# hsalehipour/XLB

Hardware: AMD Instinct MI355X
Metric: MLUPS (million lattice updates/s) D3Q19 BGK, 512^3 per GPU (higher is better)
Workload: dtype f32; 1 GPU; D3Q19 BGK FP32FP32 cavity_halfway 512x512x512 (512^3 per GPU), omega=1.0; decomposition=single GPU

## Files before the change

xlb_amd/csrc/api.hip:

```cpp
#include <cstring>

#include "api_internal.hpp"
#include "comm.hpp"

namespace xlb {

static thread_local std::string g_err;

void set_error(const char* fmt, ...) {
  char buf[1024];
  va_list ap;
  va_start(ap, fmt);
  vsnprintf(buf, sizeof(buf), fmt, ap);
  va_end(ap);
  g_err = buf;
}

int64_t opt(const xlbhip_ctx* c, const char* key, int64_t dflt) {
  auto it = c->opts.find(key);
  return it == c->opts.end() ? dflt : it->second;
}

int lattice_q(int lattice) { return lattice == XLBHIP_D2Q9 ? 9 : (lattice == XLBHIP_D3Q19 ? 19 : (lattice == XLBHIP_D3Q27 ? 27 : 0)); }
int lattice_d(int lattice) { return lattice == XLBHIP_D2Q9 ? 2 : 3; }
// ... 78 lines not shown
  int n = 0;
  XLB_HIP(hipGetDeviceCount(&n));
  XLB_REQUIRE(n > 0, "no HIP device visible");
  XLB_REQUIRE(device >= 0 && device < n, "device %d out of range (have %d)", device, n);
  XLB_HIP(hipSetDevice(device));
  xlbhip_ctx* c = new xlbhip_ctx();
  c->device = device;
  XLB_HIP(hipStreamCreateWithFlags(&c->stream, hipStreamNonBlocking));
  int prio_low = 0, prio_high = 0;
  XLB_HIP(hipDeviceGetStreamPriorityRange(&prio_low, &prio_high));
  XLB_HIP(hipStreamCreateWithPriority(&c->comm_stream, hipStreamNonBlocking, prio_high));
  XLB_HIP(hipEventCreate(&c->ev_a));
  XLB_HIP(hipEventCreate(&c->ev_b));
  XLB_HIP(hipEventCreateWithFlags(&c->ev_edge, hipEventDisableTiming));
  XLB_HIP(hipEventCreateWithFlags(&c->ev_halo, hipEventDisableTiming));
  hipDeviceProp_t p;
  XLB_HIP(hipGetDeviceProperties(&p, device));
  c->compute_units = p.multiProcessorCount;
  c->opts["vec"] = 0;
  c->opts["nt_store"] = 1;
  c->opts["nt_load"] = 1;
  c->opts["plane_pad_bytes"] = 4352;
  c->opts["block_threads"] = 256;
  c->opts["xcd_swizzle"] = 0;
  c->opts["block_tz"] = 0;
  c->opts["overlap"] = 1;
  c->opts["smagorinsky_coef_e6"] = 170000;
  c->opts["fuse2"] = 1;
  c->opts["fuse2_xseg"] = 0;
  c->opts["fuse2_clean"] = 1;
  c->opts["fuse2_cus"] = 0;
  c->opts["fuse2_strips"] = 1;
  c->opts["fuse2_rowmap"] = 0;
  c->opts["fast_bgk"] = 0;
  c->opts["exact_math"] = 0;
  c->opts["external_halo"] = 0;
  c->opts["halo_telemetry"] = 1;
  c->opts["ipc_copy"] = 1;
  c->opts["ipc_timeout_ms"] = 180000;
  c->opts["halo_skip"] = 0;
  c->opts["comm_self_test"] = 0;
  *out = c;
  return 0;
}

int xlbhip_destroy(xlbhip_ctx* c) {
  if (!c) return 0;
  (void)hipSetDevice(c->device);
  (void)hipDeviceSynchronize();
  xlbhip_comm_destroy(c);
  (void)hipEventDestroy(c->ev_a);
  (void)hipEventDestroy(c->ev_b);
  (void)hipEventDestroy(c->ev_edge);
  (void)hipEventDestroy(c->ev_halo);
  for (int i = 0; i < xlbhip_ctx::WAIT_RING; ++i) {
    if (c->ev_w0[i]) (void)hipEventDestroy(c->ev_w0[i]);
    if (c->ev_w1[i]) (void)hipEventDestroy(c->ev_w1[i]);
  }
  (void)hipStreamDestroy(c->stream);
  (void)hipStreamDestroy(c->comm_stream);
  delete c;
  return 0;
}

int xlbhip_sync(xlbhip_ctx* c) {
  XLB_REQUIRE(c, "ctx is null");
// ... 516 lines not shown
```

xlb_amd/csrc/step2_d3q19.hip:

```cpp
#include "step2_launch.hpp"

namespace xlb {

int launch_step2_d3q19_bgk(const Step2Launch& p) {
  XLB_REQUIRE(p.tile_ty == 8 && p.tile_tz == 64, "two-step kernel: only the (8 x 64) tile is built");
  if (p.halo) return p.has_bc ? launch2<D3Q19, 1, 8, 64, true>(p) : launch2<D3Q19, 0, 8, 64, true>(p);
  return p.has_bc ? launch2<D3Q19, 1, 8, 64, false>(p) : launch2<D3Q19, 0, 8, 64, false>(p);
}

int step2_build_clean(const Step2Launch& p, uint8_t* out) {
  XLB_REQUIRE(p.meta && out && p.tile_ty == 8 && (p.tile_tz == 64 || (p.tile_tz == 48 && p.halo == 0)), "clean flags: (8 x 64) / (8 x 48) tiles with meta words only");
  const size_t ghost = (size_t)p.halo * p.ny * p.nz;
  const unsigned tiles = (unsigned)(p.ny / 8) * (unsigned)(p.nz / p.tile_tz);
  const int segs = step2_eff_segments(p), swz = step2_eff_swizzle(p, tiles);
  if (p.tile_tz == 48)
    hipLaunchKernelGGL((k_step2_clean<8, 48, false>), dim3(tiles * (unsigned)segs), dim3(256), 0, p.stream, p.meta, p.tile_order, swz, segs, step2_eff_cap(p), p.x_begin,
                       p.x_count, p.nx, p.ny, p.nz, p.tile_oy, p.tile_oz, out);
  else if (p.halo)
    hipLaunchKernelGGL((k_step2_clean<8, 64, true>), dim3(tiles * (unsigned)segs), dim3(256), 0, p.stream, p.meta + ghost, p.tile_order, swz, segs, step2_eff_cap(p), p.x_begin,
                       p.x_count, p.nx, p.ny, p.nz, p.tile_oy, p.tile_oz, out);
  else
    hipLaunchKernelGGL((k_step2_clean<8, 64, false>), dim3(tiles * (unsigned)segs), dim3(256), 0, p.stream, p.meta, p.tile_order, swz, segs, step2_eff_cap(p), p.x_begin,
                       p.x_count, p.nx, p.ny, p.nz, p.tile_oy, p.tile_oz, out);
  XLB_HIP(hipGetLastError());
  return 0;
}
int step2_items(const Step2Launch& p) { return (p.ny / p.tile_ty) * (p.nz / p.tile_tz) * step2_eff_segments(p); }

}

#ifdef XLB_STEP2_TRACE
extern "C" int xlbhip_debug_step2_trace(unsigned long long* out, int n) {
  constexpr int N = xlb::TRACE_PLANES * xlb::TRACE_WAVES * xlb::TRACE_EVENTS;
  if (n < N) return N;
  if (hipDeviceSynchronize() != hipSuccess) return -1;
  return hipMemcpyFromSymbol(out, HIP_SYMBOL(xlb::g_step2_trace), sizeof(unsigned long long) * N) == hipSuccess ? 0 : -1;
}
#endif
```

xlb_amd/csrc/step2_kernel.hpp:

```cpp
#pragma once
#include "step_kernel.hpp"

namespace xlb {

#ifdef XLB_STEP2_TRACE
constexpr int TRACE_PLANES = 6, TRACE_EVENTS = 8, TRACE_WAVES = 11, TRACE_FIRST = 40, TRACE_BLOCK = 300;
static __device__ unsigned long long g_step2_trace[TRACE_PLANES * TRACE_WAVES * TRACE_EVENTS];
__device__ __forceinline__ void trace_stamp(int d, int e) {
  __builtin_amdgcn_sched_barrier(0);
  unsigned long long tm;
  asm volatile("s_memtime %0\n\ts_waitcnt lgkmcnt(0)" : "=s"(tm)::"memory");
  if (blockIdx.x == TRACE_BLOCK && d >= TRACE_FIRST && d < TRACE_FIRST + TRACE_PLANES && (threadIdx.x & 63) == 0)
    g_step2_trace[((d - TRACE_FIRST) * TRACE_WAVES + (threadIdx.x >> 6)) * TRACE_EVENTS + e] = tm;
  __builtin_amdgcn_sched_barrier(0);
}
#define XLB_TRACE(d, e) trace_stamp(d, e)
#else
#define XLB_TRACE(d, e)
#endif

template <class L>
constexpr int n_cz0() {
  int n = 0;
  for (int l = 0; l < L::Q; ++l) n += L::c(2, l) == 0 ? 1 : 0;
  return n;
}
template <class L>
constexpr int nth_cz(int cz, int k) {
  for (int l = 0; l < L::Q; ++l)
    if (L::c(2, l) == cz && k-- == 0) return l;
  return 0;
}

template <class L, int HASBC, bool SLACK = false>
struct S2Ring {
  static_assert(!SLACK || HASBC == 0, "the slack ring is the BC-free body's");
  static constexpr int group(int l) { return L::c(0, l) + 1; }
  static constexpr int gcount(int g) {
    int n = 0;
    for (int m = 0; m < L::Q; ++m) n += group(m) == g ? 1 : 0;
    return n;
  }
  static constexpr int gidx(int l) {
    int n = 0;
    for (int m = 0; m < l; ++m) n += group(m) == group(l) ? 1 : 0;
    return n;
  }
  static constexpr int glife(int g) { return (g == 0 ? (HASBC != 0 ? 2 : 1) : (g == 1 ? 2 : 3)) + (SLACK ? 1 : 0); }
  template <int life>
  static __device__ __forceinline__ int buf(int q) {
    static_assert(life >= 1 && life <= 4, "ring life");
// ... 26 lines not shown

__device__ __forceinline__ void lds_barrier() { asm volatile("s_waitcnt lgkmcnt(0)\n\ts_barrier" ::: "memory"); }

template <class L>
struct S2Meta {
  static constexpr bool WIDE = L::Q > 24;
  static constexpr unsigned KBITS = WIDE ? 3 : 4, MSHIFT = 2 * KBITS;
  static constexpr unsigned K_HWM = WIDE ? 5u : 15u;
  static __device__ __forceinline__ unsigned kind(unsigned w) { return w & ((1u << KBITS) - 1u); }
  static __device__ __forceinline__ unsigned slot(unsigned w) { return (w >> KBITS) & ((1u << KBITS) - 1u); }
  static __device__ __forceinline__ unsigned missing(unsigned w) { return WIDE ? (w >> MSHIFT) << 1 : w >> MSHIFT; }
};

__device__ __forceinline__ unsigned wave_or(unsigned v) {
  v |= (unsigned)__builtin_amdgcn_update_dpp(0, (int)v, 0x111, 0xf, 0xf, true);
  v |= (unsigned)__builtin_amdgcn_update_dpp(0, (int)v, 0x112, 0xf, 0xf, true);
  v |= (unsigned)__builtin_amdgcn_update_dpp(0, (int)v, 0x114, 0xf, 0xf, true);
  v |= (unsigned)__builtin_amdgcn_update_dpp(0, (int)v, 0x118, 0xf, 0xf, true);
  return (unsigned)__builtin_amdgcn_readlane((int)v, 15) | (unsigned)__builtin_amdgcn_readlane((int)v, 31) |
         (unsigned)__builtin_amdgcn_readlane((int)v, 47) | (unsigned)__builtin_amdgcn_readlane((int)v, 63);
}

template <class T, class S>
__device__ __forceinline__ unsigned slot_of(const StepArgs<T, S>& a, unsigned id) {
  unsigned slot = 0;
#pragma unroll
  for (int s = 0; s < MAX_FAST_BCS; ++s) {
    const unsigned sid = (unsigned)(a.ids_packed >> (8 * s)) & 0xffu;
    slot = (id == sid) ? (unsigned)s : slot;
  }
  return slot;
}

__device__ __forceinline__ void step2_seg_range(int x_begin, int x_count, int n_seg, int x_cap, int seg, int& x_lo, int& x_hi) {
  if (x_cap > 0 && n_seg >= 3) {
    const int inner = x_count - 2 * x_cap, m = n_seg - 2;
    x_lo = seg == 0 ? x_begin : x_begin + x_cap + (int)(((long)inner * (seg - 1)) / m);
    x_hi = seg == 0 ? x_begin + x_cap : (seg == n_seg - 1 ? x_begin + x_count : x_begin + x_cap + (int)(((long)inner * seg) / m));
    if (seg == n_seg - 1) x_lo = x_begin + x_count - x_cap;
  } else {
    x_lo = x_begin + (int)(((long)x_count * seg) / n_seg);
    x_hi = x_begin + (int)(((long)x_count * (seg + 1)) / n_seg);
  }
}

template <class L, class T, class S, int COLL, int HASBC, int TY, int TZ, bool SLAB, int GMAX, bool PIN, bool FAST, bool SLACK = false, int STRIPS = 0>
__device__ __forceinline__ void step2_body(const StepArgs<T, S>& a, S* lds, unsigned* ldsmeta, T* bcval, S* strip_stage = nullptr) {
  using G = S2Geom<L, HASBC, TY, TZ>;
  using R = S2Ring<L, HASBC, SLACK>;
  using M = S2Meta<L>;
  constexpr int Q = L::Q, NE = G::NE, EZ = G::EZ;
  constexpr unsigned ES = sizeof(S);
  constexpr bool SR = (STRIPS & 1) != 0, SW = (STRIPS & 2) != 0;
  static_assert(STRIPS == 0 || STRIPS == 2 || STRIPS == 3 || STRIPS == 4, "STRIPS: 0, 2 (write), 3 (read + write) or 4 (row-aligned lanes only)");
  static_assert(STRIPS == 0 || (TZ == 64 && sizeof(S) == 4), "strip buffers: (TY x 64) tiles, 4-byte store type");
  static_assert(sizeof(S) == 4, "k_step2 keeps f(t+1) as 4-byte store values in LDS");
  auto ring = [&](auto lc, int q) __attribute__((always_inline)) -> int {
    constexpr int l = decltype(lc)::value;
    constexpr int g = R::group(l), life = R::glife(g);
    return (R::gbase(g) + R::template buf<life>(q) * R::gcount(g)) * NE + R::gidx(l) * NE;
  };

  const unsigned tiles_z = (unsigned)a.nz / TZ, tiles_y = (unsigned)a.ny / TY, n_tiles = tiles_y * tiles_z;
  const unsigned seg = blockIdx.x / n_tiles, slot_in_seg = blockIdx.x % n_tiles;
  unsigned tile = slot_in_seg;
  if (a.tile_order) {
    tile = a.tile_order[slot_in_seg];
  } else if (a.xcd_swizzle) {
    const unsigned per_xcd = n_tiles / 8u;
    tile = (slot_in_seg % 8u) * per_xcd + slot_in_seg / 8u;
  }
  const int n_seg = a.x_segments > 0 ? a.x_segments : 1;
  int x_lo, x_hi;
  step2_seg_range(a.x_begin, a.x_count, n_seg, a.x_cap, (int)seg, x_lo, x_hi);
  const int ty0 = (int)(tile / tiles_z) * TY + a.tile_oy, tz0 = (int)(tile % tiles_z) * TZ + a.tile_oz;
  const int t = threadIdx.x;
  const int nx = a.nx, ny = a.ny, nz = a.nz;
  const size_t plane_cells = (size_t)ny * nz;

  if constexpr (HASBC != 0) {
    if (t < MAX_FAST_BCS * 32) {
      const unsigned s_ = (unsigned)t / 32u, l_ = (unsigned)t % 32u;
      const unsigned id_ = (unsigned)(a.ids_packed >> (8 * s_)) & 0xffu;
      bcval[t] = (l_ < 27u && id_ != 0u) ? a.bc_values[id_ * 27u + l_] : T(0);
    }
  }


  const bool act_a = t < NE;
  const int ta = act_a ? t : NE - 1;
  constexpr bool ROWMAP = (SR || (STRIPS & 4) != 0 || (HASBC == 0 && !SLACK)) && TZ == 64;
  const bool halo_wave = SR && __builtin_amdgcn_readfirstlane(t) >= G::EY * 64;
  const unsigned tile_zc = tile % tiles_z;
  const int ja = !ROWMAP ? ta / EZ : (ta < G::EY * 64 ? ta / 64 : (ta - G::EY * 64) / 2);
  const int ka = !ROWMAP ? ta % EZ : (ta < G::EY * 64 ? 1 + ta % 64 : ((ta & 1) ? EZ - 1 : 0));
  const int slot_a = ja * EZ + ka;
  int ya = ty0 - 1 + ja, za = tz0 - 1 + ka;
  ya = ya < 0 ? ya + ny : (ya >= ny ? ya - ny : ya);
  za = za < 0 ? za + nz : (za >= nz ? za - nz : za);
  unsigned Yb[3], Zb[3];
  Yb[0] = (unsigned)((ya + 1 == ny) ? 0 : ya + 1) * (unsigned)nz * ES;
  Yb[1] = (unsigned)ya * (unsigned)nz * ES;
  Yb[2] = (unsigned)((ya == 0) ? ny - 1 : ya - 1) * (unsigned)nz * ES;
  Zb[0] = (unsigned)((za + 1 == nz) ? 0 : za + 1) * ES;
  Zb[1] = (unsigned)za * ES;
  Zb[2] = (unsigned)((za == 0) ? nz - 1 : za - 1) * ES;
  if constexpr (SR) {
// ... 8 lines not shown
  }
  const unsigned cell_a = (unsigned)ya * (unsigned)nz + (unsigned)za;

  const bool act_b = t < G::NB;
  const int tb = act_b ? t : t % G::NB;
  const int jb = tb / TZ, kb = tb % TZ;
  int yb = ty0 + jb, zb = tz0 + kb;
  yb = yb >= ny ? yb - ny : yb;
  zb = zb >= nz ? zb - nz : zb;
  const unsigned cell_b = (unsigned)yb * (unsigned)nz + (unsigned)zb;
  const int ctr_b = (jb + 1) * EZ + (kb + 1);

  auto wrapx = [&](int p) __attribute__((always_inline)) {
    if constexpr (SLAB) {
      return p > x_hi ? x_hi : p;
    } else {
      p %= nx;
      return p < 0 ? p + nx : p;
    }
  };
  const ptrdiff_t pc = (ptrdiff_t)plane_cells;
  const S* pull_base = a.src;
  size_t pull_stride = a.plane_stride;
  ptrdiff_t pull_pc = pc;
  if constexpr (SR) {
    if (halo_wave) {
      pull_base = a.strips_src;
      pull_stride = a.plane_stride >> 5;
      pull_pc = pc >> 5;
    }
  }
  auto meta_load = [&](int plane, unsigned cell) __attribute__((always_inline)) -> unsigned { return (a.meta + (ptrdiff_t)plane * pc)[cell]; };

  auto finish = [&](T(&f)[Q], bool fullway) __attribute__((always_inline)) {
    if (!fullway) {
      if constexpr (COLL == XLBHIP_BGK && sizeof(T) == 4 && FAST)
        bgk_fast<L>(f, a.omega);
      else if constexpr (COLL == XLBHIP_BGK && sizeof(T) == 4)
        collide_bgk_packed<L, GMAX, PIN>(f, a.omega);
      else
        collide<L, T, COLL>(f, a.omega, a.extra);
    } else {
      static_for<Q>([&](auto lc) {
        constexpr int l = decltype(lc)::value;
        constexpr int o = opp<L>(l);
        if constexpr (l < o) {
          const T tmp = f[l];
          f[l] = f[o];
          f[o] = tmp;
        }
      });
    }
  };

  auto issue_a = [&](int x, S(&raw)[Q], unsigned w, unsigned& mall) __attribute__((always_inline)) {
    mall = 0;
    if constexpr (HASBC != 0) {
      const unsigned kind_ = M::kind(w);
      mall = wave_or((act_a && (kind_ == K_HW || kind_ == M::K_HWM)) ? M::missing(w) : 0u);
    }
    if (!act_a) return;
    int Xs[3];
    Xs[0] = SLAB ? x + 1 : ((x + 1 == nx) ? 0 : x + 1);
    Xs[1] = x;
    Xs[2] = SLAB ? x - 1 : ((x == 0) ? nx - 1 : x - 1);
    if constexpr (HASBC != 0) {
      if (mall != 0u) {
        const unsigned kind = M::kind(w);
        const unsigned m = (kind == K_HW || kind == M::K_HWM) ? M::missing(w) : 0u;
        const unsigned voff = cell_a * ES;
        static_for<Q>([&](auto lc) {
          constexpr int l = decltype(lc)::value;
// ... 10 lines not shown
    static_for<Q>([&](auto lc) {
      constexpr int l = decltype(lc)::value;
      constexpr int cx = L::c(0, l), cy = L::c(1, l), cz = L::c(2, l);
      const S* row = pull_base + (size_t)l * pull_stride + (ptrdiff_t)Xs[cx + 1] * pull_pc;
      raw[l] = ld(row, Yb[cy + 1] + Zb[cz + 1]);
    });
  };
  auto bc_regs = [&](T(&f)[Q], unsigned w, bool& fullway) __attribute__((always_inline)) {
    const unsigned kind = M::kind(w);
    if (kind == K_EQ) {
      const T* val = bcval + opaque(M::slot(w) * 32u);
      static_for<Q>([&](auto lc) { f[decltype(lc)::value] = val[decltype(lc)::value]; });
    } else if (kind == K_FW) {
      fullway = true;
    }
  };
  auto hw_apply = [&](T(&f)[Q], const T(&got)[Q], unsigned mm, unsigned w, bool any_moving) __attribute__((always_inline)) {
    if (!any_moving) {
      static_for<Q>([&](auto lc) {
        constexpr int l = decltype(lc)::value;
        const T cand = got[l] + T(0);
        f[l] = ((mm >> l) & 1u) ? cand : f[l];
      });
    } else {
      const T* val = bcval + M::slot(w) * 32u;
      const bool mov = M::kind(w) == M::K_HWM;
      static_for<Q>([&](auto lc) {
        constexpr int l = decltype(lc)::value;
        const T cand = got[l] + (mov ? val[l] : T(0));
        f[l] = ((mm >> l) & 1u) ? cand : f[l];
      });
    }
  };
  auto finish_a = [&](const S(&raw)[Q], unsigned w, unsigned mall, int q) __attribute__((always_inline)) {
    if (!act_a) return;
    T f[Q];
    static_for<Q>([&](auto lc) { f[decltype(lc)::value] = to_compute<T, S>(raw[decltype(lc)::value]); });
    bool fullway = false;
    if constexpr (HASBC != 0) {
      const unsigned kind = M::kind(w);
      const bool hw = kind == K_HW || kind == M::K_HWM;
      if (mall != 0u) {
        const unsigned mm = hw ? M::missing(w) : 0u;
        hw_apply(f, f, mm, w, __builtin_amdgcn_ballot_w64(kind == M::K_HWM) != 0ull);
      }
      if (kind != 0u) bc_regs(f, w, fullway);
    }
    finish(f, fullway);
    if (act_a) {
      S* gb[3];
      static_for<3>([&](auto gc) {
        constexpr int g = decltype(gc)::value, life = R::glife(g);
        gb[g] = lds + (R::gbase(g) + R::template buf<life>(q) * R::gcount(g)) * NE + slot_a;
      });
      static_for<Q>([&](auto lc) {
        constexpr int l = decltype(lc)::value;
        gb[R::group(l)][R::gidx(l) * NE] = to_store<S, T>(f[l]);
      });
      if constexpr (HASBC != 0) ldsmeta[(q % 3) * NE + slot_a] = w;
    }
  };

  auto phase_b_compute = [&](T(&f)[Q], int d) __attribute__((always_inline)) {
    const int q0 = d + 1;
    unsigned w = 0;
    if constexpr (HASBC != 0) w = ldsmeta[(q0 % 3) * NE + ctr_b];
    unsigned mall = 0, mm = 0;
    if constexpr (HASBC != 0) {
      const unsigned kind = M::kind(w);
      mm = (kind == K_HW || kind == M::K_HWM) ? M::missing(w) : 0u;
      mall = wave_or(mm);
    }
    if (mall == 0u) {
      const S* gb[3];
      static_for<3>([&](auto gc) {
        constexpr int g = decltype(gc)::value, life = R::glife(g);
        const int qs = q0 - (g - 1);
        gb[g] = lds + (R::gbase(g) + R::template buf<life>(qs) * R::gcount(g)) * NE;
      });
      static_for<Q>([&](auto lc) {
        constexpr int l = decltype(lc)::value;
        constexpr int cy = L::c(1, l), cz = L::c(2, l);
        f[l] = to_compute<T, S>(gb[R::group(l)][R::gidx(l) * NE + ctr_b - cy * EZ - cz]);
      });
    } else {
      T got[Q];
      static_for<Q>([&](auto lc) {
        constexpr int l = decltype(lc)::value;
        constexpr int cx = L::c(0, l), cy = L::c(1, l), cz = L::c(2, l);
        const int idx_pull = ring(lc, q0 - cx) + ctr_b - cy * EZ - cz;
        const int idx_own = ring(std::integral_constant<int, opp<L>(l)>{}, q0) + ctr_b;
        got[l] = to_compute<T, S>(lds[((mm >> l) & 1u) ? idx_own : idx_pull]);
        f[l] = got[l];
      });
      hw_apply(f, got, mm, w, __builtin_amdgcn_ballot_w64(M::kind(w) == M::K_HWM) != 0ull);
    }
    bool fullway = false;
    if constexpr (HASBC != 0) {
      if (M::kind(w) != 0u) bc_regs(f, w, fullway);
    }
    finish(f, fullway);
  };
  auto phase_b = [&](int x, int d) __attribute__((always_inline)) {
    if (!act_b) return;
    T f[Q];
    phase_b_compute(f, d);
    static_for<Q>([&](auto lc) {
      constexpr int l = decltype(lc)::value;
      S* drow = a.dst + (size_t)l * a.plane_stride + (ptrdiff_t)x * pc;
      S v[1] = {to_store<S, T>(f[l])};
      st_aligned<S, 1, true>(drow, cell_b * ES, v);
    });
    if constexpr (SW) {
      if (kb < 2 || kb >= TZ - 2) {
        constexpr int NZ1 = (Q - n_cz0<L>()) / 2, NSLOT = NZ1 + n_cz0<L>();
        const bool left = kb < 2;
        S* stg = strip_stage + (d & 1) * (NSLOT * 4 * TY) + ((left ? kb : kb - (TZ - 4)) * TY + jb) * NSLOT;
        static_for<NZ1>([&](auto kc) {
          constexpr int k = decltype(kc)::value;
          stg[k] = to_store<S, T>(left ? f[nth_cz<L>(-1, k)] : f[nth_cz<L>(1, k)]);
        });
        static_for<n_cz0<L>()>([&](auto kc) {
          constexpr int k = decltype(kc)::value;
          stg[NZ1 + k] = to_store<S, T>(f[nth_cz<L>(0, k)]);
        });
      }
    }
  };
  auto flush_strips = [&](int x, int d) __attribute__((always_inline)) {
    if constexpr (SW) {
      if (act_b) return;
      constexpr unsigned CZP = [] { unsigned m = 0; for (int l = 0; l < Q; ++l) m |= (L::c(2, l) == 1 ? 1u : 0u) << l; return m; }();
      constexpr unsigned CZM = [] { unsigned m = 0; for (int l = 0; l < Q; ++l) m |= (L::c(2, l) == -1 ? 1u : 0u) << l; return m; }();
      const int tl = t - G::NB, g = tl >> 4, i = tl & 15, r = i >> 1, e = i & 1;
      int yy = ty0 + r;
      yy = yy >= ny ? yy - ny : yy;
      const unsigned bL = tile_zc, bR = tile_zc + 1 == tiles_z ? 0u : tile_zc + 1;
      constexpr int GROUPS = (G::THREADS - G::NB) / 16;
      static_assert(GROUPS >= 1, "no idle lanes to write the strips");
#pragma unroll
      for (int rr = 0; rr * GROUPS < Q; ++rr) {
        const int l = rr * GROUPS + g;
        if (l < Q) {
          const int cz = (int)((CZP >> l) & 1u) - (int)((CZM >> l) & 1u);
          const unsigned b = cz < 0 ? bL : (cz > 0 ? bR : (e == 0 ? bL : bR));
          const unsigned j = cz != 0 ? (unsigned)e : (e == 0 ? 1u : 0u);
          constexpr int NZ1 = (Q - n_cz0<L>()) / 2, NSLOT = NZ1 + n_cz0<L>();
          constexpr unsigned CZ0 = ((1u << Q) - 1u) & ~(CZP | CZM);
          const int lane4 = cz < 0 ? e : (cz > 0 ? 2 + e : (e == 0 ? 0 : 3));
          const unsigned below = (1u << l) - 1u;
          const int k = cz < 0 ? __builtin_popcount(CZM & below) : (cz > 0 ? __builtin_popcount(CZP & below) : NZ1 + __builtin_popcount(CZ0 & below));
          const S v = strip_stage[(d & 1) * (NSLOT * 4 * TY) + (lane4 * TY + r) * NSLOT + k];
          a.strips_dst[(((ptrdiff_t)((size_t)l * a.plane_stride) + (ptrdiff_t)x * pc) >> 5) + (ptrdiff_t)(((size_t)b * (unsigned)ny + (unsigned)yy) * 2u + j)] = v;
        }
      }
    }
  };

  S raw[Q];
  unsigned w_raw = 0, mall_raw = 0;
  for (int p = -1; p <= 1; ++p) {
    if constexpr (HASBC != 0) w_raw = meta_load(wrapx(x_lo + p), cell_a);
    issue_a(wrapx(x_lo + p), raw, w_raw, mall_raw);
    if (p == -1) __syncthreads();
    finish_a(raw, w_raw, mall_raw, p + 1);
  }
  if constexpr (HASBC != 0) w_raw = meta_load(wrapx(x_lo + 2), cell_a);
  issue_a(wrapx(x_lo + 2), raw, w_raw, mall_raw);
  lds_barrier();
  for (int x = x_lo; x < x_hi; ++x) {
    const int d = x - x_lo;
    unsigned wa = 0;
    if constexpr (HASBC != 0) wa = meta_load(wrapx(x + 3), cell_a);
    XLB_TRACE(d, 0);
    phase_b(x, d);
    XLB_TRACE(d, 2);
    if constexpr (!SLACK) lds_barrier();
    XLB_TRACE(d, 3);
#if defined(XLB_STEP2_TRACE) && XLB_STEP2_TRACE == 2
    asm volatile("s_waitcnt vmcnt(0)" ::: "memory");
    XLB_TRACE(d, 4);
#endif
    finish_a(raw, w_raw, mall_raw, d + 3);
    XLB_TRACE(d, 5);
    w_raw = wa;
    if constexpr ((COLL & 3) != XLBHIP_BGK) __builtin_amdgcn_sched_barrier(0);
    issue_a(wrapx(x + 3), raw, w_raw, mall_raw);
    if (d > 0) flush_strips(x - 1, d - 1);
    XLB_TRACE(d, 6);
    lds_barrier();
    XLB_TRACE(d, 7);
  }
  if (x_hi > x_lo) flush_strips(x_hi - 1, x_hi - 1 - x_lo);
}

template <class L, class T, class S, int COLL, int HASBC, int TY, int TZ, bool SLAB, bool FAST, int STRIPS = 0>
__global__ void __attribute__((aligned(256))) __launch_bounds__((S2Geom<L, HASBC, TY, TZ>::THREADS), (S2Geom<L, HASBC, TY, TZ>::WAVES_PER_SIMD)) k_step2(const StepArgs<T, S> a) {
  using G = S2Geom<L, HASBC, TY, TZ>;
  __shared__ S lds[G::RING_PLANES * G::NE];
  __shared__ unsigned ldsmeta[HASBC ? 3 * G::NE : 1];
  __shared__ T bcval[HASBC ? MAX_FAST_BCS * 32 : 1];
  constexpr int STRIP_SLOTS = (L::Q - n_cz0<L>()) / 2 + n_cz0<L>();
  __shared__ S strip_stage[(STRIPS & 2) ? 2 * STRIP_SLOTS * 4 * TY : 1];
  static_assert(TY == 8 || (STRIPS & 2) == 0, "strip staging is laid out for 8-row tiles");
  static_assert(G::LDS_BYTES + ((STRIPS & 2) ? 2 * STRIP_SLOTS * 4 * TY * 4 : 0) <= 160 * 1024, "strip staging does not fit the LDS");
  if constexpr (HASBC != 0) {
    if (a.clean != nullptr && a.clean[blockIdx.x] != 0) {
      step2_body<L, T, S, COLL, 0, TY, TZ, SLAB, 3, true, FAST, G::SLACK, STRIPS>(a, lds, ldsmeta, bcval, strip_stage);
      return;
    }
  }
  step2_body<L, T, S, COLL, HASBC, TY, TZ, SLAB, (HASBC != 0 ? 3 : 1), HASBC != 0, FAST, false, STRIPS>(a, lds, ldsmeta, bcval, strip_stage);
}

template <int TY, int TZ, bool SLAB>
__global__ void k_step2_clean(const uint32_t* meta , const uint32_t* tile_order, int xcd_swizzle, int x_segments,
                              int x_cap, int x_begin, int x_count, int nx, int ny, int nz, int tile_oy, int tile_oz, uint8_t* clean) {
  constexpr int EY = TY + 2, EZ = TZ + 2, NE = EY * EZ;
  const unsigned tiles_z = (unsigned)nz / TZ, tiles_y = (unsigned)ny / TY, n_tiles = tiles_y * tiles_z;
  const unsigned seg = blockIdx.x / n_tiles, slot_in_seg = blockIdx.x % n_tiles;
  unsigned tile = slot_in_seg;
  if (tile_order) {
    tile = tile_order[slot_in_seg];
  } else if (xcd_swizzle) {
    const unsigned per_xcd = n_tiles / 8u;
    tile = (slot_in_seg % 8u) * per_xcd + slot_in_seg / 8u;
  }
  const int n_seg = x_segments > 0 ? x_segments : 1;
  int x_lo, x_hi;
  step2_seg_range(x_begin, x_count, n_seg, x_cap, (int)seg, x_lo, x_hi);
  const int ty0 = (int)(tile / tiles_z) * TY + tile_oy, tz0 = (int)(tile % tiles_z) * TZ + tile_oz;
  const ptrdiff_t pc = (ptrdiff_t)ny * nz;
  int dirty = 0;
  for (int p = x_lo - 1; p <= x_hi + 1; ++p) {
    int xp = p;
    if constexpr (SLAB) {
      xp = p > x_hi ? x_hi : p;
    } else {
      xp %= nx;
      xp = xp < 0 ? xp + nx : xp;
    }
    for (int t = threadIdx.x; t < NE; t += blockDim.x) {
      int y = ty0 - 1 + t / EZ, z = tz0 - 1 + t % EZ;
      y = y < 0 ? y + ny : (y >= ny ? y - ny : y);
      z = z < 0 ? z + nz : (z >= nz ? z - nz : z);
      dirty |= (meta + (ptrdiff_t)xp * pc)[(size_t)y * nz + z] != 0u;
    }
  }
  dirty = __syncthreads_or(dirty);
  if (threadIdx.x == 0) clean[blockIdx.x] = dirty ? 0 : 1;
}

}
```

xlb_amd/csrc/step2_launch.hpp:

```cpp
#pragma once
#include "step2_kernel.hpp"
#include "step_launch.hpp"

namespace xlb {

inline int step2_eff_segments(const Step2Launch& p) { return (p.x_segments > 1 && p.x_count >= 8 * p.x_segments) ? p.x_segments : 1; }
inline int step2_eff_cap(const Step2Launch& p) {
  const int n = step2_eff_segments(p);
  return (p.x_cap > 0 && n >= 3 && p.x_count - 2 * p.x_cap >= 8 * (n - 2)) ? p.x_cap : 0;
}
inline int step2_eff_swizzle(const Step2Launch& p, unsigned tiles) { return (p.xcd_swizzle && tiles % 8u == 0u) ? 1 : 0; }

template <class L, int HASBC, int TY, int TZ, bool SLAB, bool FAST, class T = float, int COLL = XLBHIP_BGK, int STRIPS = 0>
static int launch2f(const Step2Launch& p);

template <class L, int HASBC, int TY, int TZ, bool SLAB>
static int launch2(const Step2Launch& p) {
  return p.fast_bgk ? launch2f<L, HASBC, TY, TZ, SLAB, true>(p) : launch2f<L, HASBC, TY, TZ, SLAB, false>(p);
}

template <class L, int HASBC, int TY, int TZ, bool SLAB, bool FAST, class T, int COLL, int STRIPS>
static int launch2f(const Step2Launch& p) {
  static_assert(HASBC == 0 || (sizeof(T) == 4 && COLL == XLBHIP_BGK), "boundary-condition tables of the two-step kernel are fp32 / BGK");
  StepArgs<T, float> a;
  const size_t ghost = (size_t)p.halo * p.ny * p.nz;
  a.src = static_cast<const float*>(p.src) + ghost;
  a.dst = static_cast<float*>(p.dst) + ghost;
  a.bc = p.bc;
  a.miss = p.miss;
  a.meta = p.meta ? p.meta + ghost : nullptr;
  a.tile_order = p.tile_order;
  a.clean = (HASBC != 0) ? p.clean : nullptr;
  a.strips_src = (STRIPS & 1) ? static_cast<const float*>(p.strips_src) + (ghost >> 5) : nullptr;
  a.strips_dst = (STRIPS & 2) ? static_cast<float*>(p.strips_dst) + (ghost >> 5) : nullptr;
  if constexpr (STRIPS != 0) {
    XLB_REQUIRE(((STRIPS & 1) == 0 || p.strips_src) && ((STRIPS & 2) == 0 || p.strips_dst), "two-step kernel: strip buffers missing");
    XLB_REQUIRE(p.plane_stride % 32 == 0 && ((size_t)p.ny * p.nz) % 32 == 0, "two-step kernel: strip buffers need 32-element aligned planes");
  }
  a.x_segments = step2_eff_segments(p);
  a.x_cap = step2_eff_cap(p);
  a.tile_oy = p.tile_oy;
  a.tile_oz = p.tile_oz;
  a.bc_kind = p.tab_kind;
  a.bc_values = static_cast<const T*>(p.tab_values);
  a.prof_keys = nullptr;
  a.prof_vals = nullptr;
  a.n_prof = 0;
  a.dist_keys = nullptr;
  a.dist_vals = nullptr;
  a.n_dist = 0;
  a.ids_packed = p.ids_packed;
  a.kinds_packed = p.kinds_packed;
  a.n_bc = p.n_bc;
  a.plane_stride = p.plane_stride;
  a.nx = p.nx;
  a.ny = p.ny;
  a.nz = p.nz;
  a.halo = p.halo;
  a.x_begin = p.x_begin;
  a.x_count = p.x_count;
  a.nzq = p.nz;
  a.omega = static_cast<T>(p.omega);
  a.extra.force[0] = a.extra.force[1] = a.extra.force[2] = 0.0;
  a.extra.smag_cs = p.smag_cs;
  const unsigned tiles = (unsigned)(p.ny / TY) * (unsigned)(p.nz / TZ);
  a.xcd_swizzle = step2_eff_swizzle(p, tiles);
  hipLaunchKernelGGL((k_step2<L, T, float, COLL, HASBC, TY, TZ, SLAB, FAST, STRIPS>), dim3(tiles * (unsigned)a.x_segments), dim3(S2Geom<L, HASBC, TY, TZ>::THREADS), 0, p.stream, a);
  XLB_HIP(hipGetLastError());
  return 0;
}

}
```

xlb_amd/csrc/step_kernel.hpp:

```cpp
#pragma once
#include "cell.hpp"
#include "step2_plan.hpp"

#ifndef XLB_LB1
#define XLB_LB1 256
#endif

namespace xlb {

enum { K_NONE = 0, K_EQ = XLBHIP_BC_EQUILIBRIUM, K_HW = XLBHIP_BC_HALFWAY_BB, K_FW = XLBHIP_BC_FULLWAY_BB, K_DN = XLBHIP_BC_DO_NOTHING };
template <class T, class S>
struct StepArgs {
  const S* src;
  S* dst;
  const uint8_t* bc;
  const uint32_t* miss;
  const uint32_t* tile_order;
  int x_segments;
  int x_cap;
  int tile_oy, tile_oz;
  const uint32_t* meta;
  const uint8_t* clean;
  const S* strips_src;
  S* strips_dst;
  const T* bc_values;
  const uint8_t* bc_kind;
  const uint32_t* prof_keys;
  const T* prof_vals;
  int n_prof;
  const uint32_t* dist_keys;
  const float* dist_vals;
  int n_dist;
  unsigned long long ids_packed;
  unsigned kinds_packed;
  int n_bc;
  size_t plane_stride;
  int nx, ny, nz;
  int halo;
  int x_begin;
  int x_count;
  int nzq;
  CollideExtra extra;
  int xcd_swizzle;
  T omega;
};

template <class S, int N>
struct VecOf {
  typedef S aligned __attribute__((ext_vector_type(N), aligned(sizeof(S) * N)));
  typedef S shifted __attribute__((ext_vector_type(N), aligned(sizeof(S))));
};

template <class S>
__device__ __forceinline__ S ld(const S* base, unsigned boff) {
  return *reinterpret_cast<const S*>(reinterpret_cast<const char*>(base) + boff);
}
template <class S, int VEC, bool NT = false>
__device__ __forceinline__ void ld_aligned(const S* base, unsigned boff, S (&out)[VEC]) {
  if constexpr (VEC == 1) {
    if constexpr (NT)
      out[0] = __builtin_nontemporal_load(reinterpret_cast<const S*>(reinterpret_cast<const char*>(base) + boff));
    else
      out[0] = ld(base, boff);
  } else {
    typedef typename VecOf<S, VEC>::aligned V;
    V v;
    if constexpr (NT)
      v = __builtin_nontemporal_load(reinterpret_cast<const V*>(reinterpret_cast<const char*>(base) + boff));
    else
      v = *reinterpret_cast<const V*>(reinterpret_cast<const char*>(base) + boff);
#pragma unroll
    for (int k = 0; k < VEC; ++k) out[k] = v[k];
  }
}
// ... 266 lines not shown
```

xlb_amd/csrc/step_launch.hpp:

```cpp
#pragma once
#include "common.hpp"
#include "step_kernel.hpp"

namespace xlb {

struct StepLaunch {
  const void* src;
  void* dst;
  const uint8_t* bc;
  const uint32_t* miss;
  const uint8_t* tab_kind;
  const void* tab_values;
  const uint32_t* prof_keys;
  const void* prof_vals;
  int n_prof;
  const uint32_t* dist_keys;
  const float* dist_vals;
  int n_dist;
  unsigned long long ids_packed;
  unsigned kinds_packed;
  int n_bc;
  size_t plane_stride;
  int nx, ny, nz, halo;
  int x_begin, x_count;
  double omega;
  double force[3];
  double smag_cs;
  int compute_dtype, store_dtype;
  int vec;
  int has_bc;
  int flags;
  int block_threads;
  int block_tz;
  int xcd_swizzle;
  int fast_math;
  hipStream_t stream;
};

enum class Strips : int { none = 0, write = 2, read_write = 3, rowmap = 4 };

struct Step2Launch : StepLaunch {
  const uint32_t* meta = nullptr;
  const uint32_t* tile_order = nullptr;
  const uint8_t* clean = nullptr;
  const void* strips_src = nullptr;
  void* strips_dst = nullptr;
  Strips strips = Strips::none;
  int x_segments = 1;
  int x_cap = 0;
  int tile_oy = 0, tile_oz = 0;
  int tile_ty = 0, tile_tz = 0;
  int fast_bgk = 0;
};

inline int pick_vec(int compute_dtype, int nz, int requested, int collision) {
  const int vmax = (compute_dtype == XLBHIP_F32) ? 4 : 2;
  (void)collision;
  int v = requested > 0 ? requested : 1;
  if (v > vmax) v = vmax;
  if (v == 3) v = 2;
  if (nz % v != 0) v = 1;
  return v;
}

template <class L, class T, class S, int VEC, int COLL, int HASBC, int FLAGS>
int launch_typed(const StepLaunch& p) {
  StepArgs<T, S> a;
  a.src = static_cast<const S*>(p.src);
  a.dst = static_cast<S*>(p.dst);
  a.bc = p.bc;
  a.miss = p.miss;
  a.bc_kind = p.tab_kind;
  a.bc_values = static_cast<const T*>(p.tab_values);
  a.prof_keys = p.prof_keys;
  a.prof_vals = static_cast<const T*>(p.prof_vals);
  a.n_prof = p.n_prof;
  a.dist_keys = p.dist_keys;
  a.dist_vals = p.dist_vals;
  a.n_dist = p.n_dist;
  a.ids_packed = p.ids_packed;
  a.kinds_packed = p.kinds_packed;
  a.n_bc = p.n_bc;
// ... 115 lines not shown
```

xlb_amd/csrc/stepper.hip:

```cpp
#include <array>
#include <map>
#include <memory>
#include <vector>

#include "api_internal.hpp"
#include "comm.hpp"
#include "profile_tables.hpp"
#include "step_launch.hpp"

using namespace xlb;

struct FieldKey {
  const xlbhip_field* field = nullptr;
  uint64_t version = 0;
  FieldKey() = default;
  FieldKey(const xlbhip_field* f) : field(f), version(f ? f->version : 0) {}
  bool operator==(const FieldKey& o) const { return field == o.field && version == o.version; }
};
struct MetaKey {
  FieldKey bc, miss;
  bool external_halo = false;
  bool operator==(const MetaKey& o) const { return bc == o.bc && miss == o.miss && external_halo == o.external_halo; }
};

struct BcTables {
  int n_bc = 0;
  bool needs_missing = false;
  bool extended_bcs = false;
  bool has_outflow = false;
  bool has_edge_kinds = false;
  DeviceBuf tab_kind;
  unsigned long long ids_packed = 0;
  unsigned kinds_packed = 0;
  unsigned moving_mask = 0;
  DeviceBuf tab_values;
};

struct Step2Caches {
  DeviceBuf tile_order;
  int order_ty = 0, order_tz = 0;
  DeviceBuf meta;
  size_t meta_cells = 0;
  MetaKey meta_key;
  std::map<std::array<int, 3>, DeviceBuf> clean_cache;
  FieldKey scan_key;
  int scan_flag = 1;
  xlbhip_field* scratch = nullptr;

  void drop_clean() { clean_cache.clear(); }
  void forget_meta(xlbhip_ctx* c) {
    if (meta) comm_forget_buffer(c, meta.get());
    (void)meta.reset();
    meta_cells = 0;
    meta_key = MetaKey();
    drop_clean();
  }
};

struct xlbhip_stepper {
  xlbhip_ctx* ctx = nullptr;
  int lattice = 0, collision = 0, cdt = 0, sdt = 0;
  BcTables bc;
  Step2Caches pairs;
  ProfileTables prof;
  bool forced = false;
  double force[3] = {0, 0, 0};
  double smag_cs = 0.17;
  std::map<uint32_t, std::array<float, 27>> dist_host;
  DeviceBuf dist_keys;
  DeviceBuf dist_vals;
  int n_dist = 0;
};

namespace xlb {

static int launch_any(const xlbhip_stepper* s, const StepLaunch& p) {
  XLB_REQUIRE(p.n_prof == 0 || p.prof_vals, "step launch without its profile table (timestep not staged)");
// ... 68 lines not shown
  p.block_tz = (int)opt(c, "block_tz", 0);
  p.xcd_swizzle = (int)opt(c, "xcd_swizzle", 0);
  p.fast_math = opt(c, "exact_math", 0) ? 0 : 1;
  p.stream = c->stream;
  p.x_begin = 0;
  p.x_count = src->nx;
  return p;
}

static Step2Case plan_case(const xlbhip_stepper* s, const xlbhip_field* f, bool has_bc, bool edge_ext) {
  return {s->lattice, s->collision, s->cdt, s->sdt, opt(s->ctx, "exact_math", 0) ? 0 : 1, f->nx, f->ny, f->nz, f->halo,
          has_bc ? (s->bc.extended_bcs ? 2 : 1) : 0, edge_ext ? 1 : 0, s->bc.n_bc, s->bc.kinds_packed, s->bc.needs_missing ? 1 : 0};
}

static long fill_cus(const xlbhip_ctx* c) {
  const int64_t o = opt(c, "fuse2_cus", 0);
  return o > 0 ? (long)o : (c->compute_units > 0 ? c->compute_units : 256);
}

static int fuse2_segments(const xlbhip_stepper* s, const Step2Case& pc, int x_count) {
  return step2_segments(pc, x_count, fill_cus(s->ctx), (int)opt(s->ctx, "fuse2_xseg", 0), opt(s->ctx, "fuse2_clean", 1) != 0);
}

static Step2Launch make_launch2(xlbhip_stepper* s, const Step2Case& pc, const xlbhip_field* src, xlbhip_field* dst, const xlbhip_field* bcm,
                                const xlbhip_field* miss, double omega, int64_t t) {
  xlbhip_ctx* c = s->ctx;
  Step2Launch p;
  static_cast<StepLaunch&>(p) = make_launch(s, src, dst, bcm, miss, omega, t);
  p.meta = s->pairs.meta.get<uint32_t>();
  const bool clean_on = p.has_bc && opt(c, "fuse2_clean", 1) != 0;
  p.tile_order = (p.has_bc && (s->bc.needs_missing || clean_on)) ? s->pairs.tile_order.get<uint32_t>() : nullptr;
  p.x_segments = fuse2_segments(s, pc, p.x_count);
  p.x_cap = clean_on ? 8 : 0;
  const Step2Tile tile = step2_tile(s->lattice, s->collision, p.has_bc != 0);
  p.tile_ty = tile.ty;
  p.tile_tz = tile.tz;
  if (p.has_bc) {
    p.tile_oy = p.tile_ty / 2;
    p.tile_oz = p.tile_tz / 2;
  }
  p.fast_bgk = (opt(c, "fast_bgk", 0) && !opt(c, "exact_math", 0)) ? 1 : 0;
  p.xcd_swizzle = 1;
  return p;
}

template <class T>
static BcView<T> bc_view(const xlbhip_stepper* s, const void* prof_vals) {
  return {s->bc.tab_kind.get<uint8_t>(), s->bc.tab_values.get<const T>(), s->prof.keys.get<uint32_t>(), static_cast<const T*>(prof_vals), s->prof.n,
          s->dist_keys.get<uint32_t>(),  s->dist_vals.get<float>(),       s->n_dist};
}

static int outflow_aux(xlbhip_stepper* s, const xlbhip_field* src, xlbhip_field* dst, const xlbhip_field* bcm, const xlbhip_field* miss,
                       int64_t t) {
  if (!s->bc.has_outflow) return 0;
  xlbhip_ctx* c = s->ctx;
  const size_t n = dst->cells();
  const void* pv = s->prof.table_at(t);
  XLB_REQUIRE(s->prof.n == 0 || pv, "outflow pass without its profile table (timestep %lld not staged)", (long long)t);
  return by_lattice(s->lattice, [&](auto L) {
    return by_compute(s->cdt, [&](auto T) {
      using TT = decltype(T);
      hipLaunchKernelGGL((k_outflow_aux<decltype(L), TT>), blocks_for(n), BC_BLOCK, 0, c->stream, view(src), view(dst), view(bcm), view(miss), dims(dst),
                         bc_view<TT>(s, pv));
      XLB_HIP(hipGetLastError());
      return 0;
    });
  });
}

static int launch_step2(xlbhip_stepper* s, Step2Launch p) {
  if (s->lattice == XLBHIP_D3Q27 && s->collision == XLBHIP_KBC) return launch_step2_d3q27_kbc(p);
  p.clean = nullptr;
  if (p.has_bc && p.meta && opt(s->ctx, "fuse2_clean", 1)) {
    const std::array<int, 3> key = {p.x_begin, p.x_count, p.x_segments};
    auto it = s->pairs.clean_cache.find(key);
    if (it == s->pairs.clean_cache.end()) {
      DeviceBuf flags;
      XLB_HIP(flags.alloc((size_t)step2_items(p)));
      if (int rc = step2_build_clean(p, flags.get<uint8_t>())) return rc;
      it = s->pairs.clean_cache.emplace(key, std::move(flags)).first;
    }
    p.clean = it->second.get<uint8_t>();
  }
  if (s->lattice == XLBHIP_D3Q27) return launch_step2_d3q27_bgk(p);
  return p.strips != Strips::none ? launch_step2_d3q19_bgk_strips(p) : launch_step2_d3q19_bgk(p);
}

static bool ensure_strips(xlbhip_field* f) {
  if (f->strips) return true;
  const size_t bytes = f->planes * f->plane_stride * dtype_size(f->dtype) / 32 + 512;
  if (hipMalloc(&f->strips, bytes) != hipSuccess) {
    f->strips = nullptr;
    (void)hipGetLastError();
    return false;
  }
  f->strips_version = 0;
  f->strips_oz = -1;
  return true;
}

static int step_twice_edge_ext(xlbhip_stepper* s, const Step2Case& pc, Step2Launch p, const xlbhip_field* src, xlbhip_field* dst, const xlbhip_field* bcm,
                               const xlbhip_field* miss, double omega, int64_t t) {
  XLB_REQUIRE(s->pairs.scratch && s->pairs.scratch->plane_stride == src->plane_stride, "scratch field missing (can_fuse2 allocates it)");
  const int nx = src->nx;
  p.x_begin = 2;
  p.x_count = nx - 4;
  p.x_segments = fuse2_segments(s, pc, p.x_count);
// ... 475 lines not shown
```

Measured before the change: 53950 MLUPS.

## Merge periodic end segments across wrap and peel march tail with pinned collision

On a single GPU with a full periodic x range, the two boundary cap segments (first and last x_cap planes) are merged into one segment that marches across the wrap. The other segment exits early, which cuts the per-segment pipeline warm-up (the halo planes loaded before marching). The last two planes of each march are also peeled into a tail loop that skips the next plane's issue and uses a pinned collision variant. The clean-flag kernel and its cache key are updated to match the new segment ranges. The costs are more complex control flow and a load imbalance, since one segment now does twice the cap work while another does none.

```diff
diff --git a/xlb_amd/csrc/api.hip b/xlb_amd/csrc/api.hip
--- a/xlb_amd/csrc/api.hip
+++ b/xlb_amd/csrc/api.hip
@@ -134,6 +134,8 @@
   c->opts["fuse2_cus"] = 0;
   c->opts["fuse2_strips"] = 1;
   c->opts["fuse2_rowmap"] = 0;
+  c->opts["fuse2_merge_ends"] = 2;
+  c->opts["fuse2_peel_tail"] = 1;
   c->opts["fast_bgk"] = 0;
   c->opts["exact_math"] = 0;
   c->opts["external_halo"] = 0;
diff --git a/xlb_amd/csrc/step2_d3q19.hip b/xlb_amd/csrc/step2_d3q19.hip
--- a/xlb_amd/csrc/step2_d3q19.hip
+++ b/xlb_amd/csrc/step2_d3q19.hip
@@ -15,13 +15,13 @@
   const int segs = step2_eff_segments(p), swz = step2_eff_swizzle(p, tiles);
   if (p.tile_tz == 48)
     hipLaunchKernelGGL((k_step2_clean<8, 48, false>), dim3(tiles * (unsigned)segs), dim3(256), 0, p.stream, p.meta, p.tile_order, swz, segs, step2_eff_cap(p), p.x_begin,
-                       p.x_count, p.nx, p.ny, p.nz, p.tile_oy, p.tile_oz, out);
+                       p.x_count, p.nx, p.ny, p.nz, p.tile_oy, p.tile_oz, p.seg_opts, out);
   else if (p.halo)
     hipLaunchKernelGGL((k_step2_clean<8, 64, true>), dim3(tiles * (unsigned)segs), dim3(256), 0, p.stream, p.meta + ghost, p.tile_order, swz, segs, step2_eff_cap(p), p.x_begin,
-                       p.x_count, p.nx, p.ny, p.nz, p.tile_oy, p.tile_oz, out);
+                       p.x_count, p.nx, p.ny, p.nz, p.tile_oy, p.tile_oz, p.seg_opts, out);
   else
     hipLaunchKernelGGL((k_step2_clean<8, 64, false>), dim3(tiles * (unsigned)segs), dim3(256), 0, p.stream, p.meta, p.tile_order, swz, segs, step2_eff_cap(p), p.x_begin,
-                       p.x_count, p.nx, p.ny, p.nz, p.tile_oy, p.tile_oz, out);
+                       p.x_count, p.nx, p.ny, p.nz, p.tile_oy, p.tile_oz, p.seg_opts, out);
   XLB_HIP(hipGetLastError());
   return 0;
 }
diff --git a/xlb_amd/csrc/step2_kernel.hpp b/xlb_amd/csrc/step2_kernel.hpp
--- a/xlb_amd/csrc/step2_kernel.hpp
+++ b/xlb_amd/csrc/step2_kernel.hpp
@@ -17,6 +17,13 @@
 #define XLB_TRACE(d, e) trace_stamp(d, e)
 #else
 #define XLB_TRACE(d, e)
+#endif
+#if defined(XLB_STEP2_TRACE) && XLB_STEP2_TRACE == 2
+#define XLB_TRACE_DRAIN(d)                         \
+  asm volatile("s_waitcnt vmcnt(0)" ::: "memory"); \
+  XLB_TRACE(d, 4)
+#else
+#define XLB_TRACE_DRAIN(d)
 #endif
 
 template <class L>
@@ -109,16 +116,25 @@
   return slot;
 }
 
-__device__ __forceinline__ void step2_seg_range(int x_begin, int x_count, int n_seg, int x_cap, int seg, int& x_lo, int& x_hi) {
+__device__ __forceinline__ void step2_seg_range(int x_begin, int x_count, int n_seg, int x_cap, int seg, int merge, int& x_lo, int& x_hi) {
   if (x_cap > 0 && n_seg >= 3) {
     const int inner = x_count - 2 * x_cap, m = n_seg - 2;
     x_lo = seg == 0 ? x_begin : x_begin + x_cap + (int)(((long)inner * (seg - 1)) / m);
     x_hi = seg == 0 ? x_begin + x_cap : (seg == n_seg - 1 ? x_begin + x_count : x_begin + x_cap + (int)(((long)inner * seg) / m));
     if (seg == n_seg - 1) x_lo = x_begin + x_count - x_cap;
+    if (merge != 0 && (seg == 0 || seg == n_seg - 1)) {
+      const bool mine = (seg == 0) == (merge == 1);
+      x_lo = x_begin + x_count - x_cap;
+      x_hi = mine ? x_begin + x_count + x_cap : x_lo;
+    }
   } else {
     x_lo = x_begin + (int)(((long)x_count * seg) / n_seg);
     x_hi = x_begin + (int)(((long)x_count * (seg + 1)) / n_seg);
   }
+}
+__device__ __forceinline__ int step2_merge_ends(bool slab, int x_begin, int x_count, int x_cap, int nx, int seg_opts) {
+  if (slab || x_begin != 0 || x_count != nx || x_cap < 2 || (seg_opts & S2_MERGE_ENDS) == 0) return 0;
+  return (seg_opts & S2_MERGE_LAST) != 0 ? 2 : 1;
 }
 
 template <class L, class T, class S, int COLL, int HASBC, int TY, int TZ, bool SLAB, int GMAX, bool PIN, bool FAST, bool SLACK = false, int STRIPS = 0>
@@ -149,7 +165,10 @@
   }
   const int n_seg = a.x_segments > 0 ? a.x_segments : 1;
   int x_lo, x_hi;
-  step2_seg_range(a.x_begin, a.x_count, n_seg, a.x_cap, (int)seg, x_lo, x_hi);
+  constexpr bool NOWRAP = SLAB || (COLL & 3) != XLBHIP_BGK;
+  step2_seg_range(a.x_begin, a.x_count, n_seg, a.x_cap, (int)seg, step2_merge_ends(NOWRAP, a.x_begin, a.x_count, a.x_cap, a.nx, a.seg_opts), x_lo, x_hi);
+  if constexpr (!NOWRAP)
+    if (x_hi <= x_lo) return;
   const int ty0 = (int)(tile / tiles_z) * TY + a.tile_oy, tz0 = (int)(tile % tiles_z) * TZ + a.tile_oz;
   const int t = threadIdx.x;
   const int nx = a.nx, ny = a.ny, nz = a.nz;
@@ -224,12 +243,13 @@
   }
   auto meta_load = [&](int plane, unsigned cell) __attribute__((always_inline)) -> unsigned { return (a.meta + (ptrdiff_t)plane * pc)[cell]; };
 
-  auto finish = [&](T(&f)[Q], bool fullway) __attribute__((always_inline)) {
+  auto finish = [&](T(&f)[Q], bool fullway, auto pin) __attribute__((always_inline)) {
+    constexpr bool PINNED = PIN || decltype(pin)::value;
     if (!fullway) {
       if constexpr (COLL == XLBHIP_BGK && sizeof(T) == 4 && FAST)
         bgk_fast<L>(f, a.omega);
       else if constexpr (COLL == XLBHIP_BGK && sizeof(T) == 4)
-        collide_bgk_packed<L, GMAX, PIN>(f, a.omega);
+        collide_bgk_packed<L, GMAX, PINNED>(f, a.omega);
       else
         collide<L, T, COLL>(f, a.omega, a.extra);
     } else {
@@ -306,7 +326,7 @@
       });
     }
   };
-  auto finish_a = [&](const S(&raw)[Q], unsigned w, unsigned mall, int q) __attribute__((always_inline)) {
+  auto finish_a = [&](const S(&raw)[Q], unsigned w, unsigned mall, int q, auto pin) __attribute__((always_inline)) {
     if (!act_a) return;
     T f[Q];
     static_for<Q>([&](auto lc) { f[decltype(lc)::value] = to_compute<T, S>(raw[decltype(lc)::value]); });
@@ -320,7 +340,7 @@
       }
       if (kind != 0u) bc_regs(f, w, fullway);
     }
-    finish(f, fullway);
+    finish(f, fullway, pin);
     if (act_a) {
       S* gb[3];
       static_for<3>([&](auto gc) {
@@ -335,7 +355,7 @@
     }
   };
 
-  auto phase_b_compute = [&](T(&f)[Q], int d) __attribute__((always_inline)) {
+  auto phase_b_compute = [&](T(&f)[Q], int d, auto pin) __attribute__((always_inline)) {
     const int q0 = d + 1;
     unsigned w = 0;
     if constexpr (HASBC != 0) w = ldsmeta[(q0 % 3) * NE + ctr_b];
@@ -373,12 +393,12 @@
     if constexpr (HASBC != 0) {
       if (M::kind(w) != 0u) bc_regs(f, w, fullway);
     }
-    finish(f, fullway);
-  };
-  auto phase_b = [&](int x, int d) __attribute__((always_inline)) {
+    finish(f, fullway, pin);
+  };
+  auto phase_b = [&](int x, int d, auto pin) __attribute__((always_inline)) {
     if (!act_b) return;
     T f[Q];
-    phase_b_compute(f, d);
+    phase_b_compute(f, d, pin);
     static_for<Q>([&](auto lc) {
       constexpr int l = decltype(lc)::value;
       S* drow = a.dst + (size_t)l * a.plane_stride + (ptrdiff_t)x * pc;
@@ -437,35 +457,66 @@
     if constexpr (HASBC != 0) w_raw = meta_load(wrapx(x_lo + p), cell_a);
     issue_a(wrapx(x_lo + p), raw, w_raw, mall_raw);
     if (p == -1) __syncthreads();
-    finish_a(raw, w_raw, mall_raw, p + 1);
+    finish_a(raw, w_raw, mall_raw, p + 1, std::false_type{});
   }
   if constexpr (HASBC != 0) w_raw = meta_load(wrapx(x_lo + 2), cell_a);
   issue_a(wrapx(x_lo + 2), raw, w_raw, mall_raw);
   lds_barrier();
-  for (int x = x_lo; x < x_hi; ++x) {
-    const int d = x - x_lo;
-    unsigned wa = 0;
-    if constexpr (HASBC != 0) wa = meta_load(wrapx(x + 3), cell_a);
-    XLB_TRACE(d, 0);
-    phase_b(x, d);
-    XLB_TRACE(d, 2);
-    if constexpr (!SLACK) lds_barrier();
-    XLB_TRACE(d, 3);
-#if defined(XLB_STEP2_TRACE) && XLB_STEP2_TRACE == 2
-    asm volatile("s_waitcnt vmcnt(0)" ::: "memory");
-    XLB_TRACE(d, 4);
-#endif
-    finish_a(raw, w_raw, mall_raw, d + 3);
-    XLB_TRACE(d, 5);
-    w_raw = wa;
-    if constexpr ((COLL & 3) != XLBHIP_BGK) __builtin_amdgcn_sched_barrier(0);
-    issue_a(wrapx(x + 3), raw, w_raw, mall_raw);
-    if (d > 0) flush_strips(x - 1, d - 1);
-    XLB_TRACE(d, 6);
-    lds_barrier();
-    XLB_TRACE(d, 7);
-  }
-  if (x_hi > x_lo) flush_strips(x_hi - 1, x_hi - 1 - x_lo);
+  constexpr bool TAIL = !(HASBC != 0 && SW) && (COLL & 3) == XLBHIP_BGK;
+  const int x_full = TAIL && (a.seg_opts & S2_PEEL_TAIL) != 0 ? (x_hi - 2 > x_lo ? x_hi - 2 : x_lo) : x_hi;
+#define XLB_S2_TRIP(x, d, first)                                                  \
+  unsigned wa = 0;                                                                \
+  if constexpr (HASBC != 0) wa = meta_load(wrapx((x) + 3), cell_a);               \
+  XLB_TRACE(d, 0);                                                                \
+  phase_b(x, d, std::false_type{});                                               \
+  XLB_TRACE(d, 2);                                                                \
+  if constexpr (!SLACK) lds_barrier();                                            \
+  XLB_TRACE(d, 3);                                                                \
+  XLB_TRACE_DRAIN(d);                                                             \
+  finish_a(raw, w_raw, mall_raw, (d) + 3, std::false_type{});    \
+  XLB_TRACE(d, 5);                                                                \
+  w_raw = wa;                                                                     \
+  if constexpr ((COLL & 3) != XLBHIP_BGK) __builtin_amdgcn_sched_barrier(0);      \
+  issue_a(wrapx((x) + 3), raw, w_raw, mall_raw);                                  \
+  if (!(first)) flush_strips((x) - 1, (d) - 1);                                   \
+  XLB_TRACE(d, 6);                                                                \
+  lds_barrier();                                                                  \
+  XLB_TRACE(d, 7);
+  auto trip = [&](int x, int d, bool first) __attribute__((always_inline)) { XLB_S2_TRIP(x, d, first) };
+  if constexpr ((COLL & 3) != XLBHIP_BGK) {
+    static_assert(NOWRAP && !TAIL && !SW, "the KBC bodies run the plain march, without strip buffers");
+    for (int x = x_lo; x < x_hi; ++x) {
+      const int d = x - x_lo;
+      XLB_S2_TRIP(x, d, d == 0)
+    }
+  } else
+  if constexpr (NOWRAP) {
+    for (int x = x_lo; x < x_full; ++x) trip(x, x - x_lo, x == x_lo);
+    if (x_full > x_lo) flush_strips(x_full - 1, x_full - 1 - x_lo);
+  } else {
+    int xoff = 0;
+    for (int xa = x_lo; xa < x_full; xoff += nx) {
+      const int xe = x_full < xoff + nx ? x_full : xoff + nx;
+      const int x0 = xa - xoff, x1 = xe - xoff, dlo = x_lo - xoff;
+      for (int x = x0; x < x1; ++x) trip(x, x - dlo, x == x0);
+      flush_strips(x1 - 1, x1 - 1 - dlo);
+      xa = xe;
+    }
+  }
+  if constexpr (TAIL) {
+    const int toff = (!NOWRAP && x_full >= nx) ? nx : 0, t0 = x_full - toff, t1 = x_hi - toff, dlo = x_lo - toff;
+    for (int x = t0; x < t1; ++x) {
+      const int d = x - dlo;
+      phase_b(x, d, std::true_type{});
+      if (x + 2 <= t1) {
+        if constexpr (!SLACK) lds_barrier();
+        finish_a(raw, w_raw, mall_raw, d + 3, std::true_type{});
+      }
+      if (x > t0) flush_strips(x - 1, d - 1);
+      lds_barrier();
+    }
+    if (t1 > t0) flush_strips(t1 - 1, t1 - 1 - dlo);
+  }
 }
 
 template <class L, class T, class S, int COLL, int HASBC, int TY, int TZ, bool SLAB, bool FAST, int STRIPS = 0>
@@ -489,7 +540,7 @@
 
 template <int TY, int TZ, bool SLAB>
 __global__ void k_step2_clean(const uint32_t* meta , const uint32_t* tile_order, int xcd_swizzle, int x_segments,
-                              int x_cap, int x_begin, int x_count, int nx, int ny, int nz, int tile_oy, int tile_oz, uint8_t* clean) {
+                              int x_cap, int x_begin, int x_count, int nx, int ny, int nz, int tile_oy, int tile_oz, int seg_opts, uint8_t* clean) {
   constexpr int EY = TY + 2, EZ = TZ + 2, NE = EY * EZ;
   const unsigned tiles_z = (unsigned)nz / TZ, tiles_y = (unsigned)ny / TY, n_tiles = tiles_y * tiles_z;
   const unsigned seg = blockIdx.x / n_tiles, slot_in_seg = blockIdx.x % n_tiles;
@@ -502,7 +553,11 @@
   }
   const int n_seg = x_segments > 0 ? x_segments : 1;
   int x_lo, x_hi;
-  step2_seg_range(x_begin, x_count, n_seg, x_cap, (int)seg, x_lo, x_hi);
+  step2_seg_range(x_begin, x_count, n_seg, x_cap, (int)seg, step2_merge_ends(SLAB, x_begin, x_count, x_cap, nx, seg_opts), x_lo, x_hi);
+  if (x_hi <= x_lo) {
+    if (threadIdx.x == 0) clean[blockIdx.x] = 1;
+    return;
+  }
   const int ty0 = (int)(tile / tiles_z) * TY + tile_oy, tz0 = (int)(tile % tiles_z) * TZ + tile_oz;
   const ptrdiff_t pc = (ptrdiff_t)ny * nz;
   int dirty = 0;
diff --git a/xlb_amd/csrc/step2_launch.hpp b/xlb_amd/csrc/step2_launch.hpp
--- a/xlb_amd/csrc/step2_launch.hpp
+++ b/xlb_amd/csrc/step2_launch.hpp
@@ -39,6 +39,7 @@
   }
   a.x_segments = step2_eff_segments(p);
   a.x_cap = step2_eff_cap(p);
+  a.seg_opts = p.seg_opts;
   a.tile_oy = p.tile_oy;
   a.tile_oz = p.tile_oz;
   a.bc_kind = p.tab_kind;
diff --git a/xlb_amd/csrc/step_kernel.hpp b/xlb_amd/csrc/step_kernel.hpp
--- a/xlb_amd/csrc/step_kernel.hpp
+++ b/xlb_amd/csrc/step_kernel.hpp
@@ -9,6 +9,7 @@
 namespace xlb {
 
 enum { K_NONE = 0, K_EQ = XLBHIP_BC_EQUILIBRIUM, K_HW = XLBHIP_BC_HALFWAY_BB, K_FW = XLBHIP_BC_FULLWAY_BB, K_DN = XLBHIP_BC_DO_NOTHING };
+enum { S2_MERGE_ENDS = 1, S2_PEEL_TAIL = 2, S2_MERGE_LAST = 8 };
 template <class T, class S>
 struct StepArgs {
   const S* src;
@@ -40,6 +41,7 @@
   int x_begin;
   int x_count;
   int nzq;
+  int seg_opts;
   CollideExtra extra;
   int xcd_swizzle;
   T omega;
diff --git a/xlb_amd/csrc/step_launch.hpp b/xlb_amd/csrc/step_launch.hpp
--- a/xlb_amd/csrc/step_launch.hpp
+++ b/xlb_amd/csrc/step_launch.hpp
@@ -48,6 +48,7 @@
   Strips strips = Strips::none;
   int x_segments = 1;
   int x_cap = 0;
+  int seg_opts = 0;
   int tile_oy = 0, tile_oz = 0;
   int tile_ty = 0, tile_tz = 0;
   int fast_bgk = 0;
diff --git a/xlb_amd/csrc/stepper.hip b/xlb_amd/csrc/stepper.hip
--- a/xlb_amd/csrc/stepper.hip
+++ b/xlb_amd/csrc/stepper.hip
@@ -42,7 +42,7 @@
   DeviceBuf meta;
   size_t meta_cells = 0;
   MetaKey meta_key;
-  std::map<std::array<int, 3>, DeviceBuf> clean_cache;
+  std::map<std::array<int, 4>, DeviceBuf> clean_cache;
   FieldKey scan_key;
   int scan_flag = 1;
   xlbhip_field* scratch = nullptr;
@@ -177,6 +177,8 @@
   p.tile_order = (p.has_bc && (s->bc.needs_missing || clean_on)) ? s->pairs.tile_order.get<uint32_t>() : nullptr;
   p.x_segments = fuse2_segments(s, pc, p.x_count);
   p.x_cap = clean_on ? 8 : 0;
+  const int64_t merge = opt(c, "fuse2_merge_ends", 2);
+  p.seg_opts = (merge ? S2_MERGE_ENDS : 0) | (merge == 2 ? S2_MERGE_LAST : 0) | (opt(c, "fuse2_peel_tail", 1) ? S2_PEEL_TAIL : 0);
   const Step2Tile tile = step2_tile(s->lattice, s->collision, p.has_bc != 0);
   p.tile_ty = tile.ty;
   p.tile_tz = tile.tz;
@@ -217,7 +219,7 @@
   if (s->lattice == XLBHIP_D3Q27 && s->collision == XLBHIP_KBC) return launch_step2_d3q27_kbc(p);
   p.clean = nullptr;
   if (p.has_bc && p.meta && opt(s->ctx, "fuse2_clean", 1)) {
-    const std::array<int, 3> key = {p.x_begin, p.x_count, p.x_segments};
+    const std::array<int, 4> key = {p.x_begin, p.x_count, p.x_segments, p.seg_opts & (S2_MERGE_ENDS | S2_MERGE_LAST)};
     auto it = s->pairs.clean_cache.find(key);
     if (it == s->pairs.clean_cache.end()) {
       DeviceBuf flags;
```

New measurement: 54700 MLUPS (median of 6 runs). 1.4% higher.
